# TusKANNy/seismic

Hardware: AMD Instinct MI355X
Metric: queries/sec + mean latency (µs) at fixed recall@10 vs exact, SPLADE-v3 MSMARCO (higher is better)
Workload: dtype f32

## Files before the change

include/seismic_hip_testing.h:

```cpp
#ifndef SEISMIC_HIP_TESTING_H
#define SEISMIC_HIP_TESTING_H
#include "seismic_hip.h"
#ifdef __cplusplus
extern "C" {
#endif

uint32_t sgpu_debug_host_threads(void);
uint32_t sgpu_debug_chunk_bounds(uint32_t nq, uint32_t chunk_min, uint32_t chunk_max, uint32_t lanes_free, uint32_t* bounds);
sgpu_status sgpu_debug_pack_forward(const sgpu_index* idx, uint8_t* out_fwd, uint64_t cap, uint64_t* out_doc_ref,
                                    uint64_t* out_bytes);
sgpu_status sgpu_debug_row_dir(const sgpu_index* idx, uint32_t* out, uint64_t cap_words, uint64_t* n_words, uint32_t* n_buckets);
sgpu_status sgpu_debug_plan(const sgpu_index* idx, const uint64_t* q_off, const uint32_t* comps, const float* vals,
                            uint32_t nq, uint32_t query_cut, uint32_t* order_out, uint32_t* out3);
sgpu_status sgpu_debug_device_plan(sgpu_index* idx, const uint64_t* q_off, const uint32_t* comps, const float* vals,
                                   uint32_t nq, uint32_t query_cut, uint32_t* order_out, uint32_t* out3);
void sgpu_debug_call_timing(double* buf8);
uint32_t sgpu_debug_coop_trace(sgpu_index* idx, uint64_t* out, uint32_t cap);

#ifdef __cplusplus
}
#endif
#endif
```

seismic_amd/csrc/abi.cpp:

```cpp
#include <algorithm>
#include <chrono>
#include <cstdlib>
#include <mutex>
#include <new>
#include <string>
#include <thread>
#include <vector>

#include "host_index.hpp"

struct sgpu_batch;

namespace sgpu {
struct Lane;
sgpu_status device_index_upload(const HostIndex& h, int device, DeviceIndex** out);
sgpu_status device_index_clone(const DeviceIndex* src, int device, DeviceIndex** out);
void device_index_free(DeviceIndex* d);
uint64_t device_index_bytes(const DeviceIndex* d);
Lane* lane_acquire(DeviceIndex* d);
Lane* lane_try_acquire(DeviceIndex* d);
bool call_enter(DeviceIndex* d);
void call_exit(DeviceIndex* d);
void lane_release(DeviceIndex* d, Lane* l);
Lane* lane_main(DeviceIndex* d);
sgpu_batch** lane_scratch(Lane* l);
sgpu_status batch_create(DeviceIndex* d, Lane* lane, uint64_t dim, const uint64_t* q_off, const uint32_t* comps,
                         const float* vals, uint32_t nq, uint32_t k_max, sgpu_batch** out);
void batch_free(sgpu_batch* b);
sgpu_status batch_run(DeviceIndex* d, Lane* lane, sgpu_batch* b, const sgpu_search_params& sp, uint32_t mode,
                      int sync, sgpu_launch_stats* stats);
sgpu_status batch_sync(DeviceIndex* d, sgpu_launch_stats* stats);
sgpu_status batch_fetch(DeviceIndex* d, Lane* lane, sgpu_batch* b, uint32_t k, float* out_scores, uint64_t* out_ids,
                        uint32_t* out_n);
sgpu_status batch_fetch_stats(DeviceIndex* d, sgpu_batch* b, uint32_t* out);
sgpu_status staged_launch(DeviceIndex* d, Lane* lane, uint64_t dim, const uint64_t* q_off, const uint32_t* comps,
                          const float* vals, uint32_t nq, uint32_t q_base, const sgpu_search_params& sp, sgpu_batch** slot,
                          uint32_t followed,
                          const FilterRef* flt);
sgpu_status staged_finish(DeviceIndex* d, Lane* lane, sgpu_batch* b, float* out_scores, uint64_t* out_ids, uint32_t* out_n);
sgpu_status summary_distances(DeviceIndex* d, const HostIndex& h, uint32_t list, const uint32_t* comps,
                              const float* vals, uint32_t nnz, float* out_dots, uint32_t* out_nb);
int device_count();
double*& call_timing();
bool device_plan_applies(const DeviceIndex* d, const sgpu_search_params& sp);
sgpu_status debug_device_plan(DeviceIndex* d, const uint64_t* q_off, const uint32_t* comps, const float* vals, uint32_t nq,
                              uint32_t query_cut, uint32_t* order_out, uint32_t* out3);
sgpu_status debug_plan(const HostIndex& h, const uint64_t* q_off, const uint32_t* comps, const float* vals, uint32_t nq,
                       uint32_t query_cut, uint32_t* order_out, uint32_t* out3);
uint32_t coop_trace_dump(DeviceIndex* d, uint64_t* out, uint32_t cap);
const DeviceIndex* batch_replica(const sgpu_batch* b);
sgpu_status device_index_set_knn(DeviceIndex* d, const std::vector<uint32_t>& knn, uint32_t knn_dim);
sgpu_status build_knn_on_device(DeviceIndex* d, HostIndex& h, uint32_t nknn);
sgpu_status exact_search_device(sgpu_index* idx, uint32_t replica, const uint64_t* q_off, const uint32_t* comps,
                                const float* vals, uint32_t nq, uint32_t k, float* out_scores, uint64_t* out_ids,
                                uint32_t* out_n, const sgpu_filter* filter);
sgpu_status filter_create(sgpu_index* idx, const uint32_t* doc_ids, uint64_t n, sgpu_filter** out);
const sgpu_index* filter_index(const sgpu_filter* f);
const uint32_t* filter_host_bits(const sgpu_filter* f);
uint64_t filter_count(const sgpu_filter* f);
uint64_t filter_device_bytes(const sgpu_filter* f);
void filter_destroy(sgpu_filter* f);
bool filter_build_times(const sgpu_filter* f, uint32_t replica, double* out2);
}

using namespace sgpu;

extern "C" {

const char* sgpu_last_error(void) { return last_error().c_str(); }
uint32_t sgpu_abi_version(void) { return 4; }

sgpu_status sgpu_device_count(int32_t* n) {
  if (!n) return fail(SGPU_EINVAL, "null argument");
  *n = device_count();
  if (*n <= 0) {
    *n = 0;
    return fail(SGPU_EDEVICE, "no HIP device visible");
  }
  return SGPU_OK;
}

sgpu_status sgpu_index_create(const sgpu_index_desc* desc, sgpu_index** out) {
  if (!desc || !out) return fail(SGPU_EINVAL, "null argument");
  sgpu_index* ix = new (std::nothrow) sgpu_index();
  if (!ix) return fail(SGPU_ENOMEM, "out of memory");
  sgpu_status st = host_index_from_desc(*desc, &ix->host);
  if (st != SGPU_OK) {
    delete ix;
    return st;
  }
  *out = ix;
  return SGPU_OK;
}

sgpu_status sgpu_index_build(uint32_t comp_width, uint64_t n_docs, uint64_t dim, const uint64_t* offsets,
                             const void* comps, const float* vals, const sgpu_build_config* cfg,
                             sgpu_index** out) {
  if (!offsets || !cfg || !out || (offsets[n_docs] && (!comps || !vals))) return fail(SGPU_EINVAL, "null argument");
  sgpu_index* ix = new (std::nothrow) sgpu_index();
  if (!ix) return fail(SGPU_ENOMEM, "out of memory");
  sgpu_status st = build_host_index(comp_width, n_docs, dim, offsets, comps, vals, *cfg, &ix->host);
  if (st != SGPU_OK) {
// ... 168 lines not shown
  DeviceIndex* d = replica_of(idx, replica);
  if (!d) return SGPU_EDEVICE;
  return batch_create(d, lane_main(d), idx->host.dim, q_off, comps, vals, nq, k_max, out);
}

sgpu_status sgpu_batch_create(sgpu_index* idx, const uint64_t* q_off, const uint32_t* comps, const float* vals,
                              uint32_t nq, uint32_t k_max, sgpu_batch** out) {
  return sgpu_batch_create_on(idx, 0, q_off, comps, vals, nq, k_max, out);
}

sgpu_status sgpu_batch_run(sgpu_index* idx, sgpu_batch* batch, const sgpu_search_params* params, int32_t sync,
                           sgpu_launch_stats* stats) {
  if (!idx || !batch || !params) return fail(SGPU_EINVAL, "null argument");
  DeviceIndex* d = replica_of_batch(idx, batch);
  if (!d) return SGPU_EINVAL;
  return batch_run(d, nullptr, batch, *params, 0 , sync, stats);
}

sgpu_status sgpu_batch_run_counted(sgpu_index* idx, sgpu_batch* batch, const sgpu_search_params* params,
                                   sgpu_launch_stats* stats) {
  if (!idx || !batch || !params) return fail(SGPU_EINVAL, "null argument");
  DeviceIndex* d = replica_of_batch(idx, batch);
  if (!d) return SGPU_EINVAL;
  return batch_run(d, nullptr, batch, *params, 2 , 1, stats);
}

sgpu_status sgpu_batch_sync(sgpu_index* idx, sgpu_launch_stats* stats) {
  if (!idx) return fail(SGPU_EINVAL, "null argument");
  for (size_t i = idx->replicas.size(); i-- > 1;) {
    sgpu_status st = batch_sync(idx->replicas[i], nullptr);
    if (st != SGPU_OK) return st;
  }
  return batch_sync(idx->dev, stats);
}

sgpu_status sgpu_batch_fetch(sgpu_index* idx, sgpu_batch* batch, uint32_t k, float* out_scores,
                             uint64_t* out_doc_ids, uint32_t* out_n) {
  if (!idx || !batch || !out_scores || !out_doc_ids || !out_n) return fail(SGPU_EINVAL, "null argument");
  DeviceIndex* d = replica_of_batch(idx, batch);
  if (!d) return SGPU_EINVAL;
  return batch_fetch(d, nullptr, batch, k, out_scores, out_doc_ids, out_n);
}

sgpu_status sgpu_batch_fetch_stats(sgpu_index* idx, sgpu_batch* batch, uint32_t* out_counters) {
  if (!idx || !batch || !out_counters) return fail(SGPU_EINVAL, "null argument");
  DeviceIndex* d = replica_of_batch(idx, batch);
  if (!d) return SGPU_EINVAL;
  return batch_fetch_stats(d, batch, out_counters);
}

void sgpu_batch_destroy(sgpu_batch* batch) { batch_free(batch); }

static uint32_t chunk_jobs(uint32_t nq, uint32_t chunk_min, uint32_t chunk_max) {
  return chunk_min && nq >= 2 * chunk_min ? std::min<uint32_t>(chunk_max, nq / chunk_min) : 1u;
}
static void chunk_bounds(uint32_t nq, uint32_t n_jobs, uint32_t j, uint32_t* q0, uint32_t* q1) {
  *q0 = (uint32_t)((uint64_t)nq * j / n_jobs);
  *q1 = (uint32_t)((uint64_t)nq * (j + 1) / n_jobs);
}

static sgpu_status search_shard(DeviceIndex* d, uint64_t dim, const uint64_t* q_off, const uint32_t* comps,
                                const float* vals, uint32_t nq, uint32_t q_base, const sgpu_search_params& params,
                                float* out_scores, uint64_t* out_doc_ids, uint32_t* out_n, const FilterRef* flt) {
  static const uint32_t chunk_min = [] {
    const char* v = std::getenv("SGPU_CHUNK_MIN");
    return v && *v ? (uint32_t)std::strtoul(v, nullptr, 10) : 0xffffffffu;
  }();
  struct Job {
    Lane* lane;
    uint32_t q0, q1;
  };
  static const uint32_t chunk_max_env = [] {
    const char* v = std::getenv("SGPU_CHUNK_MAX");
    const uint32_t n = v && *v ? (uint32_t)std::strtoul(v, nullptr, 10) : 0u;
    return n > 8 ? 8u : n;
  }();
  struct InFlight {
    DeviceIndex* d;
    bool shared;
    explicit InFlight(DeviceIndex* d_) : d(d_), shared(call_enter(d_)) {}
    ~InFlight() { call_exit(d); }
  } in_flight(d);
  const uint32_t chunk_max = chunk_max_env ? chunk_max_env : ((in_flight.shared || device_plan_applies(d, params)) ? 2u : 4u);
  Job jobs[8];
  const uint32_t cmin = chunk_min != 0xffffffffu ? chunk_min : (device_plan_applies(d, params) ? 1300u : 600u);
  uint32_t n_jobs = chunk_jobs(nq, cmin, chunk_max);
  std::vector<uint64_t> off;
  if (n_jobs > 1) {
    try {
      off.resize((size_t)nq / 2 + 2);
    } catch (const std::exception&) {
      n_jobs = 1;
    }
  }
  jobs[0].lane = lane_acquire(d);
  for (uint32_t j = 1; j < n_jobs; ++j) {
    jobs[j].lane = lane_try_acquire(d);
    if (!jobs[j].lane) {
      n_jobs = j;
      break;
    }
  }
  const uint32_t k = params.k;
  sgpu_status st = SGPU_OK;
  std::string msg;
  uint32_t launched = 0;
  if (n_jobs > 1) {
    uint32_t max_nnz = 0;
    st = q_off[0] != 0 ? fail(SGPU_EINVAL, "q_off[0] must be 0") : validate_query_offsets(q_off, nq, q_base, &max_nnz);
    if (st != SGPU_OK) msg = last_error();
  }
  for (uint32_t j = 0; j < n_jobs && st == SGPU_OK; ++j) {
    Job& jb = jobs[j];
    chunk_bounds(nq, n_jobs, j, &jb.q0, &jb.q1);
    const uint64_t* qo = q_off;
    if (n_jobs > 1 && jb.q0 != 0) {
      for (uint32_t q = jb.q0; q <= jb.q1; ++q) off[q - jb.q0] = q_off[q] - q_off[jb.q0];
      qo = off.data();
    }
    st = staged_launch(d, jb.lane, dim, qo, comps ? comps + q_off[jb.q0] : nullptr, vals ? vals + q_off[jb.q0] : nullptr,
                       jb.q1 - jb.q0, q_base + jb.q0, params, lane_scratch(jb.lane), j + 1 < n_jobs ? 2u : (in_flight.shared ? 1u : 0u),
                       flt);
    if (st == SGPU_OK) ++launched;
    else msg = last_error();
  }
  for (uint32_t j = 0; j < launched; ++j) {
    Job& jb = jobs[j];
    const sgpu_status fs = staged_finish(d, jb.lane, *lane_scratch(jb.lane), out_scores + (size_t)jb.q0 * k,
                                         out_doc_ids + (size_t)jb.q0 * k, out_n + jb.q0);
    if (fs != SGPU_OK && st == SGPU_OK) {
      st = fs;
      msg = last_error();
    }
  }
  for (uint32_t j = 0; j < n_jobs; ++j) lane_release(d, jobs[j].lane);
  if (st != SGPU_OK) last_error() = msg;
  return st;
}

}

static sgpu_status batch_search(sgpu_index* idx, const uint64_t* q_off, const uint32_t* comps, const float* vals,
                                uint32_t nq, const sgpu_search_params* params, float* out_scores,
                                uint64_t* out_doc_ids, uint32_t* out_n, const sgpu_filter* filter) {
  if (!idx || !params || !q_off || !out_scores || !out_doc_ids || !out_n) return fail(SGPU_EINVAL, "null argument");
  if (params->k == 0) return fail(SGPU_EINVAL, "k must be > 0 (KHeap::new asserts, reference src/utils.rs:23)");
  if (idx->replicas.empty()) return fail(SGPU_EDEVICE, "index is not uploaded to a device (call sgpu_index_upload)");
  if (q_off[nq] && (!comps || !vals)) return fail(SGPU_EINVAL, "null argument");
  const uint32_t n_rep = (uint32_t)idx->replicas.size();
  if (n_rep == 1) {
    const FilterRef fr{filter, 0};
    return search_shard(idx->dev, idx->host.dim, q_off, comps, vals, nq, 0, *params, out_scores, out_doc_ids, out_n,
                        filter ? &fr : nullptr);
  }
  if (nq < 2 * n_rep) {
    const uint32_t r = idx->next_replica.fetch_add(1, std::memory_order_relaxed) % n_rep;
    const FilterRef fr{filter, r};
    return search_shard(idx->replicas[r], idx->host.dim, q_off, comps, vals, nq, 0, *params, out_scores, out_doc_ids, out_n,
                        filter ? &fr : nullptr);
  }
  {
    uint32_t max_nnz = 0;
    if (q_off[0] != 0) return fail(SGPU_EINVAL, "q_off[0] must be 0");
    const sgpu_status vst = validate_query_offsets(q_off, nq, 0, &max_nnz);
    if (vst != SGPU_OK) return vst;
  }
  const uint32_t k = params->k;
  try {
    std::vector<sgpu_status> sts(n_rep, SGPU_OK);
    std::vector<std::string> msgs(n_rep);
    std::vector<std::vector<uint64_t>> offs(n_rep);
    for (uint32_t r = 0; r < n_rep; ++r) {
      const uint32_t q0 = (uint32_t)((uint64_t)nq * r / n_rep), q1 = (uint32_t)((uint64_t)nq * (r + 1) / n_rep);
      offs[r].resize(q1 - q0 + 1);
      for (uint32_t q = q0; q <= q1; ++q) offs[r][q - q0] = q_off[q] - q_off[q0];
    }
    auto shard = [&](uint32_t r) {
      const uint32_t q0 = (uint32_t)((uint64_t)nq * r / n_rep), q1 = (uint32_t)((uint64_t)nq * (r + 1) / n_rep);
      try {
        const FilterRef fr{filter, r};
        sts[r] = search_shard(idx->replicas[r], idx->host.dim, offs[r].data(), comps ? comps + q_off[q0] : nullptr,
                              vals ? vals + q_off[q0] : nullptr, q1 - q0, q0, *params, out_scores + (size_t)q0 * k,
                              out_doc_ids + (size_t)q0 * k, out_n + q0, filter ? &fr : nullptr);
        if (sts[r] != SGPU_OK) msgs[r] = last_error();
      } catch (const std::exception&) {
        sts[r] = SGPU_ENOMEM;
      }
    };
    std::vector<std::thread> threads;
// ... 72 lines not shown
  if (breakdown_us) slot = phases;
  const uint32_t k = params->k;
  sgpu_status st = SGPU_OK;
  const auto t0 = std::chrono::steady_clock::now();
  for (uint32_t q = 0; q < nq && st == SGPU_OK; ++q) {
    if (q_off[q + 1] < q_off[q] || q_off[q + 1] - q_off[q] > 0xffffffffull) {
      st = fail(SGPU_EINVAL, "query offsets must be monotone (query %u)", q);
      break;
    }
    const auto tq = per_query_us ? std::chrono::steady_clock::now() : t0;
    st = sgpu_search(idx, comps ? comps + q_off[q] : nullptr, vals ? vals + q_off[q] : nullptr,
                     (uint32_t)(q_off[q + 1] - q_off[q]), params, out_scores + (size_t)q * k,
                     out_doc_ids + (size_t)q * k, out_n + q);
    if (per_query_us) per_query_us[q] = std::chrono::duration<double, std::micro>(std::chrono::steady_clock::now() - tq).count();
  }
  const double total = std::chrono::duration<double, std::micro>(std::chrono::steady_clock::now() - t0).count();
  slot = saved;
  if (mean_us) *mean_us = nq ? total / nq : 0.0;
  if (breakdown_us)
    for (int i = 0; i < 8; ++i) breakdown_us[i] = nq ? phases[i] / nq : 0.0;
  return st;
}

sgpu_status sgpu_search_sequential(sgpu_index* idx, const uint64_t* q_off, const uint32_t* comps, const float* vals,
                                   uint32_t nq, const sgpu_search_params* params, float* out_scores,
                                   uint64_t* out_doc_ids, uint32_t* out_n, double* mean_us, double* breakdown_us) {
  return sgpu_search_sequential_timed(idx, q_off, comps, vals, nq, params, out_scores, out_doc_ids, out_n, mean_us,
                                      breakdown_us, nullptr);
}

static bool test_hooks_on() {
  const char* t = std::getenv("SGPU_TEST_HOOKS");
  return t && *t && *t != '0';
}
#define SGPU_HOOK_OR(ret)                                                                            \
  if (!test_hooks_on()) {                                                                            \
    (void)fail(SGPU_EINVAL, "%s is a test hook: set SGPU_TEST_HOOKS=1 (include/seismic_hip_testing.h)", __func__); \
    return ret;                                                                                      \
  }

uint32_t sgpu_debug_host_threads(void) {
  SGPU_HOOK_OR(0u);
  return (uint32_t)host_threads();
}

uint32_t sgpu_debug_chunk_bounds(uint32_t nq, uint32_t chunk_min, uint32_t chunk_max, uint32_t lanes_free, uint32_t* bounds) {
  SGPU_HOOK_OR(0u);
  uint32_t n_jobs = chunk_jobs(nq, chunk_min, chunk_max < 1 ? 1 : (chunk_max > 8 ? 8 : chunk_max));
  if (lanes_free >= 1 && n_jobs > lanes_free) n_jobs = lanes_free;
  for (uint32_t j = 0; j < n_jobs; ++j) chunk_bounds(nq, n_jobs, j, bounds + 2 * j, bounds + 2 * j + 1);
  return n_jobs;
}

sgpu_status sgpu_debug_pack_forward(const sgpu_index* idx, uint8_t* out_fwd, uint64_t cap, uint64_t* out_doc_ref, uint64_t* out_bytes) {
  SGPU_HOOK_OR(SGPU_EINVAL);
  if (!idx || !out_bytes) return fail(SGPU_EINVAL, "null argument");
  try {
    std::vector<uint8_t> raw, fwd;
    std::vector<uint64_t> off16, dref;
    pack_dvb_raw_flags(idx->host, &raw);
    pack_record_offsets(idx->host, raw, 128 / 16, &off16);
    *out_bytes = std::max<uint64_t>(off16[idx->host.n_docs] * 16, 16);
    if (!out_fwd) return SGPU_OK;
    if (cap < *out_bytes || !out_doc_ref) return fail(SGPU_EINVAL, "buffer too small");
    pack_records(idx->host, raw, off16, &fwd);
    pack_doc_refs(idx->host, raw, off16, &dref);
    std::memcpy(out_fwd, fwd.data(), fwd.size());
    std::memcpy(out_doc_ref, dref.data(), dref.size() * 8);
  } catch (const std::bad_alloc&) {
    return fail(SGPU_ENOMEM, "out of host memory");
  }
  return SGPU_OK;
}

sgpu_status sgpu_debug_row_dir(const sgpu_index* idx, uint32_t* out, uint64_t cap_words, uint64_t* n_words, uint32_t* n_buckets) {
  SGPU_HOOK_OR(SGPU_EINVAL);
  if (!idx || !n_words || !n_buckets) return fail(SGPU_EINVAL, "null argument");
  try {
    std::vector<uint16_t> mid;
    std::vector<uint32_t> dir;
    pack_row_mid(idx->host, &mid);
    *n_buckets = 0;
    if (!pack_row_dir(idx->host, mid, &dir, n_buckets)) *n_buckets = 0;
    *n_words = dir.size();
    if (!out) return SGPU_OK;
    if (cap_words < dir.size()) return fail(SGPU_EINVAL, "buffer too small");
    std::memcpy(out, dir.data(), dir.size() * 4);
  } catch (const std::bad_alloc&) {
    return fail(SGPU_ENOMEM, "out of host memory");
  }
  return SGPU_OK;
}

sgpu_status sgpu_debug_plan(const sgpu_index* idx, const uint64_t* q_off, const uint32_t* comps, const float* vals, uint32_t nq,
                            uint32_t query_cut, uint32_t* order_out, uint32_t* out3) {
  SGPU_HOOK_OR(SGPU_EINVAL);
  if (!idx || !q_off || !order_out || !out3) return fail(SGPU_EINVAL, "null argument");
  return debug_plan(idx->host, q_off, comps, vals, nq, query_cut, order_out, out3);
}

sgpu_status sgpu_debug_device_plan(sgpu_index* idx, const uint64_t* q_off, const uint32_t* comps, const float* vals, uint32_t nq,
                                   uint32_t query_cut, uint32_t* order_out, uint32_t* out3) {
  SGPU_HOOK_OR(SGPU_EINVAL);
  if (!idx || !q_off || !order_out || !out3) return fail(SGPU_EINVAL, "null argument");
  return debug_device_plan(idx->dev, q_off, comps, vals, nq, query_cut, order_out, out3);
}
// ... 60 lines not shown
```

seismic_amd/csrc/common.hpp:

```cpp
#pragma once
#include <cstdarg>
#include <cstdint>
#include <cstdio>
#include <cstring>
#include <string>

#include "../../include/seismic_hip.h"

namespace sgpu {

std::string& last_error();
sgpu_status fail(sgpu_status st, const char* fmt, ...) __attribute__((format(printf, 2, 3)));

int default_host_threads(int omp_max_threads);
}
#ifdef _OPENMP
#include <omp.h>
#endif
namespace sgpu {
inline int host_threads() {
#ifdef _OPENMP
  return default_host_threads(omp_get_max_threads());
#else
  return 1;
#endif
}

inline float f16_to_f32(uint16_t h) {
  const uint32_t sign = (uint32_t)(h & 0x8000u) << 16;
  const uint32_t em = h & 0x7fffu;
  uint32_t bits;
  if (em >= 0x7c00u) {
    bits = sign | 0x7f800000u | ((em & 0x3ffu) << 13);
  } else if (em >= 0x0400u) {
    bits = sign | ((em << 13) + 0x38000000u);
  } else if (em == 0) {
    bits = sign;
  } else {
    float f = (float)em * 5.9604644775390625e-08f;
    uint32_t fb;
    std::memcpy(&fb, &f, 4);
    bits = sign | fb;
  }
  float f;
  std::memcpy(&f, &bits, 4);
  return f;
}

inline uint16_t f32_to_f16_sat(float f) {
  uint32_t x;
  std::memcpy(&x, &f, 4);
  const uint16_t sign = (uint16_t)((x >> 16) & 0x8000u);
  x &= 0x7fffffffu;
  if (x > 0x7f800000u) return (uint16_t)(sign | 0x7e00u);
  if (x >= 0x477ff000u) return (uint16_t)(sign | 0x7bffu);
  if (x < 0x38800000u) {
    float a;
    std::memcpy(&a, &x, 4);
    float r = __builtin_nearbyintf(a * 16777216.0f);
    return (uint16_t)(sign | (uint16_t)r);
  }
  const uint32_t lsb = (x >> 13) & 1u;
  x += 0xfffu + lsb;
  return (uint16_t)(sign | (uint16_t)((x - 0x38000000u) >> 13));
}

inline int32_t total_key(float f) {
// ... 27 lines not shown
```

seismic_amd/csrc/device_index.hip:

```cpp
#include <hip/hip_runtime.h>

#include <algorithm>
#include <atomic>
#include <chrono>
#include <cmath>
#include <condition_variable>
#include <cstdlib>
#include <cstring>
#include <mutex>
#include <unordered_map>
#include <vector>

#include "device_types.hpp"
#include "filter.hpp"
#include "host_index.hpp"

namespace sgpu {

hipError_t run_u16_dense(const LaunchArgs& a, int* occupancy);
hipError_t run_u16_packed(const LaunchArgs& a, int* occupancy);
hipError_t run_u32_split(const LaunchArgs& a, int* occupancy);
hipError_t run_u32_packed(const LaunchArgs& a, int* occupancy);
hipError_t run_u32_hash(const LaunchArgs& a, int* occupancy);
hipError_t run_u16_dense_u8(const LaunchArgs& a, int* occupancy);
// ... 426 lines not shown
    if (e != hipSuccess) return bail(fail(SGPU_EDEVICE, "hipMemcpyPeerAsync %d -> %d failed: %s", src->device, device, hipGetErrorString(e)));
  }
  if (hipStreamSynchronize(d->main.stream) != hipSuccess) return bail(fail(SGPU_EDEVICE, "peer copy failed"));
  *out = d;
  return SGPU_OK;
}

}

struct sgpu_batch_plan {
  uint32_t query_cut = 0;
  uint32_t dots_cap = 1;
  uint32_t max_nb = 0;
  uint32_t max_list_nb = 1;
  std::vector<uint32_t> order;
  bool hash_ok = true;
};

struct sgpu_batch {
  std::vector<uint64_t> h_off;
  std::vector<uint32_t> h_off32;
  std::vector<uint32_t> h_comp;
  std::vector<float> h_val;
  std::vector<sgpu_batch_plan> plans;
  int device = -1;
  const sgpu::DeviceIndex* owner = nullptr;
  uint32_t nq = 0, k_max = 0, max_nnz = 0;
  uint64_t cap_nq = 0, cap_nnz = 0, cap_slab = 0;
  uint32_t* q_off = nullptr;
  uint32_t* q_comp = nullptr;
  float* q_val = nullptr;
  uint32_t* q_order = nullptr;
  uint32_t* h_order = nullptr;
  uint32_t order_cut = 0xffffffffu;
  float* out_scores = nullptr;
  uint64_t* out_ids = nullptr;
  uint32_t* out_n = nullptr;
  uint32_t* out_stats = nullptr;
  uint32_t* status = nullptr;
  size_t status_off = 0;
  bool staged = false;
  uint8_t* arena_dev = nullptr;
  uint8_t* arena_host = nullptr;
  uint8_t* arena_host_dev = nullptr;
  bool direct_out = false;
  uint32_t done_seq = 0;
  bool direct_in = false;
  uint32_t queue_base = 0;
  size_t arena_cap = 0, in_bytes = 0, out_off = 0, out_bytes = 0;
  uint32_t* queue_dev = nullptr;
  uint32_t device_plan_cut = 0xffffffffu;
  bool followed = false;
  bool plan_identity = false;
};

namespace sgpu {

}
extern char** environ;
namespace sgpu {
struct EnvCache {
  uint64_t fp = 0;
  int n = 0;
  struct E {
    const char* name;
    const char* val;
  } e[96];
};
static thread_local EnvCache tl_env;
static void env_refresh() {
  uint64_t h = 1469598103934665603ull;
  for (char** p = environ; p && *p; ++p) h = (h ^ (uint64_t)(uintptr_t)*p) * 1099511628211ull;
  if (h != tl_env.fp || tl_env.n == 0) {
    tl_env.fp = h;
    tl_env.n = 0;
  }
}
static const char* env_get(const char* name) {
  EnvCache& c = tl_env;
  for (int i = 0; i < c.n; ++i)
    if (c.e[i].name == name) return c.e[i].val;
  const char* v = std::getenv(name);
  if (c.n < (int)(sizeof(c.e) / sizeof(c.e[0]))) c.e[c.n++] = EnvCache::E{name, v};
  return v;
}
static uint32_t env_u32(const char* name, uint32_t dflt) {
  const char* v = env_get(name);
  if (!v || !*v) return dflt;
  return (uint32_t)std::strtoul(v, nullptr, 10);
}
static bool hooks_on() {
  const char* v = env_get("SGPU_TEST_HOOKS");
  return v && *v && *v != '0';
}
static void hook_ignored(const char* name) {
  static std::atomic<bool> said{false};
  const char* v = env_get(name);
  if (v && *v && !said.exchange(true))
    std::fprintf(stderr, "seismic_hip: %s is a test hook and is ignored unless SGPU_TEST_HOOKS=1 is set (further ignored hooks are not reported)\n", name);
}
static uint32_t hook_u32(const char* name, uint32_t dflt) {
  if (hooks_on()) return env_u32(name, dflt);
  hook_ignored(name);
  return dflt;
}
static const char* hook_get(const char* name) {
// ... 201 lines not shown
    pl.order.resize(2 * (size_t)nq);
    for (uint32_t i = 0; i < nq; ++i) pl.order[i] = (uint32_t)keys[i];
    pl.hash_ok = d->view.dim < (1u << 24) && d->comp_width == 4 && d->value_type == SGPU_VAL_F16 && !hook_u32("SGPU_NO_HASH", 0);
    if (pl.hash_ok) {
      std::vector<uint32_t> stamp(kHashSlots, 0xffffffffu);
      uint32_t epoch = 0;
      for (uint32_t q = 0; q < nq && pl.hash_ok; ++q) {
        const uint64_t a = h_off[q], e = h_off[q + 1];
        uint32_t seed = kHashSeeds;
        if (e - a <= kHashSlots / 4)
          for (uint32_t s = 0; s < kHashSeeds && seed == kHashSeeds; ++s) {
            const uint32_t mult = hash_mult(s);
            bool clash = false;
            for (uint64_t i = a; i < e && !clash; ++i) {
              uint32_t& slot = stamp[hash_slot(h_comp[i], mult)];
              clash = slot == epoch;
              slot = epoch;
            }
            ++epoch;
            if (!clash) seed = s;
          }
        if (seed == kHashSeeds) pl.hash_ok = false;
        pl.order[(size_t)nq + q] = seed & (kHashSeeds - 1);
      }
    }
  } catch (const std::bad_alloc&) {
    return fail(SGPU_ENOMEM, "out of host memory planning a query batch");
  }
  return SGPU_OK;
}

sgpu_status debug_plan(const HostIndex& h, const uint64_t* q_off, const uint32_t* comps, const float* vals, uint32_t nq,
                       uint32_t query_cut, uint32_t* order_out, uint32_t* out3) {
  DeviceIndex d;
  d.comp_width = h.comp_width;
  d.view.dim = (uint32_t)h.dim;
  d.list_nb.resize(h.dim);
  d.list_np.resize(h.dim);
  for (uint64_t c = 0; c < h.dim; ++c) {
    d.list_nb[c] = (uint32_t)(h.list_block_start[c + 1] - h.list_block_start[c]);
    d.list_np[c] = (uint32_t)(h.block_post_start[h.list_block_start[c + 1]] - h.block_post_start[h.list_block_start[c]]);
  }
  sgpu_batch_plan pl;
  env_refresh();
  const sgpu_status st = make_plan(&d, q_off, comps, vals, nq, query_cut, &pl);
  if (st != SGPU_OK) return st;
  for (uint32_t i = 0; i < nq; ++i) order_out[i] = pl.order[i];
  out3[0] = pl.dots_cap;
  out3[1] = pl.max_nb;
  out3[2] = pl.max_list_nb;
  return SGPU_OK;
}

bool device_plan_applies(const DeviceIndex* d, const sgpu_search_params& sp) {
  const bool hash_family = d->comp_width == 4 && d->value_type == SGPU_VAL_F16 && d->view.dim < (1u << 24);
  const char* v = std::getenv("SGPU_DEVICE_PLAN");
  return sp.query_cut >= 1 && sp.query_cut <= kDevicePlanCutMax && !sp.first_sorted && !hash_family && !(v && *v == '0');
}

sgpu_status debug_device_plan(DeviceIndex* d, const uint64_t* q_off, const uint32_t* comps, const float* vals, uint32_t nq,
                              uint32_t query_cut, uint32_t* order_out, uint32_t* out3) {
  if (!d) return fail(SGPU_EDEVICE, "index is not uploaded to a device");
  if (nq == 0 || nq > kDevicePlanMaxQueries || query_cut == 0 || query_cut > kDevicePlanCutMax)
    return fail(SGPU_EINVAL, "the device plans 1 ... %u queries at query_cut 1 ... %u", (unsigned)kDevicePlanMaxQueries, (unsigned)kDevicePlanCutMax);
  HIP_TRY(hipSetDevice(d->device));
  const uint64_t nnz = q_off[nq];
  uint32_t n2 = 2;
  while (n2 < nq) n2 <<= 1;
  std::vector<uint32_t> off32((size_t)nq + 1);
  for (uint32_t q = 0; q <= nq; ++q) off32[q] = (uint32_t)q_off[q];
  const size_t o_comp = al16_((size_t)(nq + 1) * 4), o_val = o_comp + al16_(nnz * 4), o_keys = o_val + al16_(nnz * 4),
               o_max = o_keys + (size_t)n2 * 8, o_order = o_max + 16, total = o_order + (size_t)nq * 4;
  uint8_t* buf = nullptr;
  if (hipMalloc((void**)&buf, total) != hipSuccess) return fail(SGPU_ENOMEM, "hipMalloc of %zu bytes failed", total);
  hipError_t e = hipMemcpy(buf, off32.data(), (size_t)(nq + 1) * 4, hipMemcpyHostToDevice);
  if (e == hipSuccess && nnz) e = hipMemcpy(buf + o_comp, comps, nnz * 4, hipMemcpyHostToDevice);
  if (e == hipSuccess && nnz) e = hipMemcpy(buf + o_val, vals, nnz * 4, hipMemcpyHostToDevice);
  if (e == hipSuccess) e = hipMemset(buf + o_max, 0, 16);
  if (e == hipSuccess)
    e = launch_device_plan(d->view, (const uint32_t*)buf, (const uint32_t*)(buf + o_comp), (const float*)(buf + o_val), nq, query_cut,
                           (uint64_t*)(buf + o_keys), (uint32_t*)(buf + o_max), (uint32_t*)(buf + o_order), d->main.stream);
  if (e == hipSuccess) e = hipStreamSynchronize(d->main.stream);
  if (e == hipSuccess) e = hipMemcpy(order_out, buf + o_order, (size_t)nq * 4, hipMemcpyDeviceToHost);
  if (e == hipSuccess) e = hipMemcpy(out3, buf + o_max, 12, hipMemcpyDeviceToHost);
  (void)hipFree(buf);
  if (e != hipSuccess) return fail(SGPU_EDEVICE, "device plan failed: %s", hipGetErrorString(e));
  return SGPU_OK;
}

static sgpu_status plan_for(DeviceIndex* d, sgpu_batch* b, uint32_t query_cut, const sgpu_batch_plan** out) {
  for (const auto& pl : b->plans)
    if (pl.query_cut == query_cut) {
      *out = &pl;
      return SGPU_OK;
    }
  if (b->staged) return fail(SGPU_EINVAL, "a staged batch is planned when it is staged");
  sgpu_batch_plan pl;
  sgpu_status st = make_plan(d, b->h_off.data(), b->h_comp.data(), b->h_val.data(), b->nq, query_cut, &pl);
  if (st != SGPU_OK) return st;
  try {
    b->plans.push_back(std::move(pl));
  } catch (const std::bad_alloc&) {
    return fail(SGPU_ENOMEM, "out of host memory planning a query batch");
  }
  *out = &b->plans.back();
  return SGPU_OK;
}

static bool coop_by_size(const DeviceIndex* d, uint32_t nq) {
  const char* v = env_get("SGPU_COOP_MAX_NQ");
// ... 426 lines not shown
                        uint32_t* out_n) {
  if (!d || !b) return fail(SGPU_EINVAL, "null index/batch");
  if (k == 0 || k > b->k_max) return fail(SGPU_EINVAL, "k out of range for this batch");
  if (!lane) lane = &d->main;
  HIP_TRY(hipSetDevice(d->device));
  if (b->nq == 0) {
    HIP_TRY(hipStreamSynchronize(lane->stream));
    return SGPU_OK;
  }
  if (k == b->k_max) {
    HIP_TRY(hipMemcpyAsync(out_scores, b->out_scores, (size_t)b->nq * k * 4, hipMemcpyDeviceToHost, lane->stream));
    HIP_TRY(hipMemcpyAsync(out_ids, b->out_ids, (size_t)b->nq * k * 8, hipMemcpyDeviceToHost, lane->stream));
  } else {
    HIP_TRY(hipMemcpy2DAsync(out_scores, (size_t)k * 4, b->out_scores, (size_t)b->k_max * 4, (size_t)k * 4, b->nq,
                             hipMemcpyDeviceToHost, lane->stream));
    HIP_TRY(hipMemcpy2DAsync(out_ids, (size_t)k * 8, b->out_ids, (size_t)b->k_max * 8, (size_t)k * 8, b->nq,
                             hipMemcpyDeviceToHost, lane->stream));
  }
  HIP_TRY(hipMemcpyAsync(out_n, b->out_n, (size_t)b->nq * 4, hipMemcpyDeviceToHost, lane->stream));
  HIP_TRY(hipStreamSynchronize(lane->stream));
  return coop_check_board(d, lane);
}

sgpu_status batch_fetch_stats(DeviceIndex* d, sgpu_batch* b, uint32_t* out) {
  if (!d || !b || !out) return fail(SGPU_EINVAL, "null index/batch/out");
  HIP_TRY(hipSetDevice(d->device));
  HIP_TRY(hipStreamSynchronize(d->main.stream));
  if (b->nq) HIP_TRY(hipMemcpy(out, b->out_stats, (size_t)b->nq * STATS_WORDS * 4, hipMemcpyDeviceToHost));
  return SGPU_OK;
}

uint32_t coop_trace_dump(DeviceIndex* d, uint64_t* out, uint32_t cap) {
  if (!d) return 0;
  (void)hipSetDevice(d->device);
  Lane* lanes[DeviceIndex::kPool + 1];
  int nl = 0;
  lanes[nl++] = &d->main;
  for (Lane& l : d->pool) lanes[nl++] = &l;
  for (int i = 0; i < nl; ++i) {
    Lane* l = lanes[i];
    if (!l->coop || !l->coop_trace_n) continue;
    (void)hipStreamSynchronize(l->stream);
    const uint32_t n = std::min<uint32_t>(cap, l->coop_trace_n);
    if (hipMemcpy(out, l->coop + l->coop_trace_off, (size_t)n * 8, hipMemcpyDeviceToHost) != hipSuccess) return 0;
    return n;
  }
  return 0;
}

static inline size_t al16(size_t x) { return (x + 15) & ~(size_t)15; }

sgpu_status staged_launch(DeviceIndex* d, Lane* lane, uint64_t dim, const uint64_t* q_off, const uint32_t* comps,
                          const float* vals, uint32_t nq, uint32_t q_base, const sgpu_search_params& sp, sgpu_batch** slot,
                          uint32_t followed, const FilterRef* flt) {
  if (!d) return fail(SGPU_EDEVICE, "index is not uploaded to a device (call sgpu_index_upload)");
  if (sp.k == 0) return fail(SGPU_EINVAL, "k must be > 0 (KHeap::new asserts, reference src/utils.rs:23)");
  if (sp.k > 1024) return fail(SGPU_ELIMIT, "k = %u exceeds the heap limit of 1024", sp.k);
  uint32_t max_nnz = 0;
  PhaseClock pc;
  env_refresh();
  if (!q_off || q_off[0] != 0) return fail(SGPU_EINVAL, "q_off[0] must be 0");
  sgpu_status st = validate_query_offsets(q_off, nq, q_base, &max_nnz);
  if (st != SGPU_OK) return st;
  if (q_off[nq] && (!comps || !vals)) return fail(SGPU_EINVAL, "null query arrays");
  bool validated = false;
  HIP_TRY(hipSetDevice(d->device));
  const uint64_t nnz = q_off[nq];
  const uint32_t k = sp.k;
  const size_t o_fix = 16, o_off = 32, o_comp = o_off + al16((size_t)(nq + 1) * 4), o_val = o_comp + al16(nnz * 4),
               o_order = o_val + al16(nnz * 4), o_status = o_order + al16((size_t)nq * 8),
               in_bytes = o_status + 16;
  const size_t r_n = in_bytes, r_sc = r_n + al16((size_t)nq * 4), r_id = r_sc + al16((size_t)nq * k * 4),
               total = r_id + al16((size_t)nq * k * 8);
  sgpu_batch* b = *slot;
  if (b && (!b->staged || b->owner != d || b->arena_cap < total)) {
    HIP_TRY(hipStreamSynchronize(lane->stream));
    batch_free(b);
    b = nullptr;
    *slot = nullptr;
  }
  if (!b) {
    b = new (std::nothrow) sgpu_batch();
    if (!b) return fail(SGPU_ENOMEM, "out of host memory");
    b->staged = true;
    b->device = d->device;
    b->owner = d;
    b->arena_cap = std::max<size_t>(std::min<size_t>(total * 5 / 2, total + ((size_t)64 << 20)), 1 << 16);
    if (hipMalloc((void**)&b->arena_dev, b->arena_cap) != hipSuccess ||
        hipHostMalloc((void**)&b->arena_host, b->arena_cap, hipHostMallocMapped | hipHostMallocCoherent) != hipSuccess) {
      batch_free(b);
      return fail(SGPU_ENOMEM, "allocation of a %zu-byte staging arena failed", b->arena_cap);
    }
    if (hipHostGetDevicePointer((void**)&b->arena_host_dev, b->arena_host, 0) != hipSuccess) b->arena_host_dev = nullptr;
    *slot = b;
    if (hook_raw("SGPU_DEBUG_ALLOC")) std::fprintf(stderr, "sgpu alloc: arena %p..%p\n", (void*)b->arena_dev, (void*)(b->arena_dev + b->arena_cap));
  }
  b->nq = nq;
  b->k_max = k;
  b->max_nnz = max_nnz;
  b->in_bytes = in_bytes;
  b->out_off = r_n;
  b->out_bytes = total - r_n;
  if (nq == 0) {
    b->status_off = o_status;
    return SGPU_OK;
  }
  const uint32_t direct_max = hook_u32("SGPU_DIRECT_OUT_MAX", 16);
  const uint32_t qn = std::max<uint32_t>(4, (max_nnz + 3u) & ~3u);
  const uint32_t cut = std::min<uint32_t>(sp.query_cut, qn);
  try {
    b->plans.clear();
    b->plans.emplace_back();
  } catch (const std::bad_alloc&) {
    return fail(SGPU_ENOMEM, "out of host memory planning a query batch");
  }
  b->device_plan_cut = 0xffffffffu;
  b->followed = followed != 0;
  b->plan_identity = false;
  {
    const bool hash_family = d->comp_width == 4 && d->value_type == SGPU_VAL_F16 && d->view.dim < (1u << 24);
    uint32_t seen = 0;
    if (nq >= kDevicePlanMinQueries && nq <= kDevicePlanMaxQueries && cut >= 1 && cut <= kDevicePlanCutMax && !sp.first_sorted &&
        !hash_family && env_u32("SGPU_DEVICE_PLAN", 1) && !hook_u32("SGPU_NO_LPT", 0)) {
      std::lock_guard<std::mutex> lock(d->mu);
      auto it = d->plan_dots_seen.find(cut);
      if (it != d->plan_dots_seen.end()) seen = it->second;
    }
    if (seen && nq <= direct_max) seen = 0;
    if (!seen) {
      st = validate_queries(dim, q_off, comps, vals, nq, &max_nnz, q_base);
      if (st != SGPU_OK) return st;
      validated = true;
    }
    if (seen) {
      sgpu_batch_plan& pl = b->plans.back();
      pl.query_cut = cut;
      pl.dots_cap = std::max(seen, std::max<uint32_t>(d->max_nb, 1));
      pl.max_nb = 0;
      pl.max_list_nb = std::max<uint32_t>(d->max_nb, 1);
      pl.hash_ok = false;
      pl.order.clear();
      b->device_plan_cut = cut;
      b->plan_identity = followed == 2 && hook_u32("SGPU_PLAN_IDENTITY", 1) != 0;
    } else {
      st = make_plan(d, q_off, comps, vals, nq, cut, &b->plans.back());
      if (st != SGPU_OK) return st;
      std::lock_guard<std::mutex> lock(d->mu);
      uint32_t& v = d->plan_dots_seen[cut];
      v = std::max(v, b->plans.back().dots_cap);
    }
  }
  pc.lap(0);
  uint8_t* hs = b->arena_host;
  std::memset(hs, 0, 16);
  uint32_t* h32 = (uint32_t*)(hs + o_off);
  for (uint32_t q = 0; q <= nq; ++q) h32[q] = (uint32_t)q_off[q];
  if (nnz) {
    std::memcpy(hs + o_comp, comps, nnz * 4);
    std::memcpy(hs + o_val, vals, nnz * 4);
  }
  if (b->device_plan_cut == 0xffffffffu) std::memcpy(hs + o_order, b->plans.back().order.data(), (size_t)nq * 8);
  std::memset(hs + o_status, 0, 16);
  std::memset(hs + o_fix, 0, 16);
  const uint32_t direct_in_on = env_u32("SGPU_DIRECT_IN", 1);
  b->direct_out = b->arena_host_dev != nullptr && nq <= direct_max;
  b->direct_in = b->direct_out && direct_in_on != 0;
  uint8_t* in_base = b->direct_in ? b->arena_host_dev : b->arena_dev;
  b->queue_dev = b->direct_in ? lane->queue + 16 : (uint32_t*)b->arena_dev;
  b->queue_base = 0;
  b->q_off = (uint32_t*)(in_base + o_off);
  b->q_comp = (uint32_t*)(in_base + o_comp);
  b->q_val = (float*)(in_base + o_val);
  b->q_order = (uint32_t*)(in_base + o_order);
  b->order_cut = cut;
  uint8_t* out_base = b->direct_out ? b->arena_host_dev : b->arena_dev;
  b->out_n = (uint32_t*)(out_base + r_n);
  b->out_scores = (float*)(out_base + r_sc);
  b->out_ids = (uint64_t*)(out_base + r_id);
  b->out_stats = nullptr;
  b->status_off = b->direct_out ? o_fix : o_status;
  b->status = (uint32_t*)(out_base + b->status_off);
  pc.lap(1);
  if (b->direct_in) {
    if (lane->queue_dirty) {
      HIP_TRY(hipMemsetAsync(lane->queue + 16, 0, 4, lane->stream));
      lane->queue_pos = 0;
      lane->queue_dirty = false;
    }
    b->queue_base = lane->queue_pos;
  } else {
    HIP_TRY(hipMemcpyAsync(b->arena_dev, hs, in_bytes, hipMemcpyHostToDevice, lane->stream));
    if (!validated) {
      st = validate_queries(dim, q_off, comps, vals, nq, &max_nnz, q_base);
      if (st != SGPU_OK) {
        const std::string msg = last_error();
        (void)hipStreamSynchronize(lane->stream);
        last_error() = msg;
        return st;
      }
      validated = true;
    }
  }
  const DevView* view = &d->view;
  if (flt && flt->f) {
    const FilterDeviceView* fv = nullptr;
    st = filter_view(flt->f, flt->replica, &fv);
    if (st != SGPU_OK) {
      const std::string msg = last_error();
      (void)hipStreamSynchronize(lane->stream);
      last_error() = msg;
      return st;
    }
    view = &fv->view;
    HIP_TRY(hipSetDevice(d->device));
  }
  if (!b->direct_in && b->device_plan_cut != 0xffffffffu && !b->plan_identity) {
    HIP_TRY(launch_device_plan(*view, b->q_off, b->q_comp, b->q_val, nq, cut, (uint64_t*)(b->arena_dev + r_n),
                               (uint32_t*)(b->arena_dev + o_status) + 1, b->q_order, lane->stream));
  }
  pc.lap(2);
  hipError_t he = hipSuccess;
  {
    std::lock_guard<std::mutex> lock(d->mu);
    LaunchArgs a{};
    st = configure(d, lane, b, sp, MODE_SEARCH, &a, view);
    if (st == SGPU_OK) he = launch_search(a);
    if (b->direct_in) {
      if (st == SGPU_OK && he == hipSuccess) lane->queue_pos += nq + a.grid;
      else lane->queue_dirty = true;
    }
  }
  pc.lap(3);
  if (st == SGPU_OK && he == hipSuccess && !b->direct_out)
    he = hipMemcpyAsync(hs + o_status, b->arena_dev + o_status, 16 + b->out_bytes, hipMemcpyDeviceToHost, lane->stream);
  pc.lap(4);
  if (st != SGPU_OK || he != hipSuccess) {
    (void)hipStreamSynchronize(lane->stream);
    if (st == SGPU_OK) st = fail(SGPU_EDEVICE, "launch of the search failed: %s", hipGetErrorString(he));
    return st;
  }
  return SGPU_OK;
}

sgpu_status staged_finish(DeviceIndex* d, Lane* lane, sgpu_batch* b, float* out_scores, uint64_t* out_ids, uint32_t* out_n) {
  HIP_TRY(hipSetDevice(d->device));
  PhaseClock pc;
  {
    const volatile uint32_t* done = (b && b->done_seq) ? (const volatile uint32_t*)(b->arena_host + b->status_off + 4) : nullptr;
    const hipError_t we = wait_lane(lane->stream, b ? b->nq : 0, done, b ? b->done_seq : 0u);
    if (we != hipSuccess) lane->queue_dirty = true;
    HIP_TRY(we);
  }
  pc.lap(5);
  if (!b || b->nq == 0) return SGPU_OK;
  {
    const sgpu_status cs = coop_report(d, lane, *(const volatile uint32_t*)(b->arena_host + b->status_off));
    if (cs != SGPU_OK) {
      lane->queue_dirty = true;
      return cs;
    }
  }
  if (b->device_plan_cut != 0xffffffffu) {
    const uint32_t need = ((const volatile uint32_t*)(b->arena_host + b->status_off))[1];
    std::lock_guard<std::mutex> lock(d->mu);
    uint32_t& v = d->plan_dots_seen[b->device_plan_cut];
    v = std::max(v, need);
  }
  const size_t nq = b->nq, k = b->k_max;
  const uint8_t* r = b->arena_host + b->out_off;
  std::memcpy(out_n, r, nq * 4);
  std::memcpy(out_scores, r + al16(nq * 4), nq * k * 4);
  std::memcpy(out_ids, r + al16(nq * 4) + al16(nq * k * 4), nq * k * 8);
  pc.lap(6);
  return SGPU_OK;
}

sgpu_status summary_distances(DeviceIndex* d, const HostIndex& h, uint32_t list, const uint32_t* comps,
                              const float* vals, uint32_t nnz, float* out_dots, uint32_t* out_nb) {
  if (!d) return fail(SGPU_EDEVICE, "index is not uploaded to a device (call sgpu_index_upload)");
  if (list >= h.dim) return fail(SGPU_EINVAL, "list %u >= dim", list);
  const uint32_t nb = (uint32_t)(h.list_block_start[list + 1] - h.list_block_start[list]);
  *out_nb = nb;
  if (nb == 0 || nnz == 0) {
    for (uint32_t i = 0; i < nb; ++i) out_dots[i] = 0.0f;
    return SGPU_OK;
  }
  const uint64_t q_off[2] = {0, nnz};
  sgpu_batch* b = nullptr;
  sgpu_status st = batch_create(d, &d->main, h.dim, q_off, comps, vals, 1, 1, &b);
  if (st != SGPU_OK) return st;
  sgpu_search_params sp{};
  sp.k = 1;
  sp.query_cut = list;
  sp.heap_factor = 0;
// ... 91 lines not shown
```

Baseline: 1.753 million.

## Segment large query calls and plan later chunks on host

Large query batches are now split into segments of at most 8×16384 queries, and each segment is cut into chunks bounded by a maximum chunk size, so device-plan limits are respected. Chunks after the first now build their plan on the host instead of using the device plan, unless an environment variable selects otherwise. The device-plan applicability check is refactored into a helper that returns the cached dot capacity, and plan_dots_seen is only updated for batches large enough. This adds host planning work on later chunks and changes lane concurrency for very large calls.

```diff
diff --git a/include/seismic_hip_testing.h b/include/seismic_hip_testing.h
--- a/include/seismic_hip_testing.h
+++ b/include/seismic_hip_testing.h
@@ -7,6 +7,9 @@
 
 uint32_t sgpu_debug_host_threads(void);
 uint32_t sgpu_debug_chunk_bounds(uint32_t nq, uint32_t chunk_min, uint32_t chunk_max, uint32_t lanes_free, uint32_t* bounds);
+uint32_t sgpu_debug_call_bounds(uint32_t nq, uint32_t chunk_min, uint32_t chunk_max, uint32_t lanes_free, uint32_t first_pm,
+                                uint32_t* bounds, uint32_t cap);
+uint32_t sgpu_debug_lane_chunk(sgpu_index* idx, uint32_t lane, uint32_t* info4, uint32_t* order_out, uint32_t cap);
 sgpu_status sgpu_debug_pack_forward(const sgpu_index* idx, uint8_t* out_fwd, uint64_t cap, uint64_t* out_doc_ref,
                                     uint64_t* out_bytes);
 sgpu_status sgpu_debug_row_dir(const sgpu_index* idx, uint32_t* out, uint64_t cap_words, uint64_t* n_words, uint32_t* n_buckets);
diff --git a/seismic_amd/csrc/abi.cpp b/seismic_amd/csrc/abi.cpp
--- a/seismic_amd/csrc/abi.cpp
+++ b/seismic_amd/csrc/abi.cpp
@@ -36,18 +36,19 @@
 sgpu_status staged_launch(DeviceIndex* d, Lane* lane, uint64_t dim, const uint64_t* q_off, const uint32_t* comps,
                           const float* vals, uint32_t nq, uint32_t q_base, const sgpu_search_params& sp, sgpu_batch** slot,
                           uint32_t followed,
-                          const FilterRef* flt);
+                          const FilterRef* flt, uint32_t chunk);
 sgpu_status staged_finish(DeviceIndex* d, Lane* lane, sgpu_batch* b, float* out_scores, uint64_t* out_ids, uint32_t* out_n);
 sgpu_status summary_distances(DeviceIndex* d, const HostIndex& h, uint32_t list, const uint32_t* comps,
                               const float* vals, uint32_t nnz, float* out_dots, uint32_t* out_nb);
 int device_count();
 double*& call_timing();
-bool device_plan_applies(const DeviceIndex* d, const sgpu_search_params& sp);
+uint32_t device_plan_dots(DeviceIndex* d, const sgpu_search_params& sp, uint32_t nq, uint32_t cut);
 sgpu_status debug_device_plan(DeviceIndex* d, const uint64_t* q_off, const uint32_t* comps, const float* vals, uint32_t nq,
                               uint32_t query_cut, uint32_t* order_out, uint32_t* out3);
 sgpu_status debug_plan(const HostIndex& h, const uint64_t* q_off, const uint32_t* comps, const float* vals, uint32_t nq,
                        uint32_t query_cut, uint32_t* order_out, uint32_t* out3);
 uint32_t coop_trace_dump(DeviceIndex* d, uint64_t* out, uint32_t cap);
+uint32_t debug_lane_chunk(DeviceIndex* d, uint32_t lane, uint32_t* info4, uint32_t* order_out, uint32_t cap);
 const DeviceIndex* batch_replica(const sgpu_batch* b);
 sgpu_status device_index_set_knn(DeviceIndex* d, const std::vector<uint32_t>& knn, uint32_t knn_dim);
 sgpu_status build_knn_on_device(DeviceIndex* d, HostIndex& h, uint32_t nknn);
@@ -322,16 +323,29 @@
 void sgpu_batch_destroy(sgpu_batch* batch) { batch_free(batch); }
 
 static uint32_t chunk_jobs(uint32_t nq, uint32_t chunk_min, uint32_t chunk_max) {
-  return chunk_min && nq >= 2 * chunk_min ? std::min<uint32_t>(chunk_max, nq / chunk_min) : 1u;
-}
-static void chunk_bounds(uint32_t nq, uint32_t n_jobs, uint32_t j, uint32_t* q0, uint32_t* q1) {
-  *q0 = (uint32_t)((uint64_t)nq * j / n_jobs);
-  *q1 = (uint32_t)((uint64_t)nq * (j + 1) / n_jobs);
-}
-
-static sgpu_status search_shard(DeviceIndex* d, uint64_t dim, const uint64_t* q_off, const uint32_t* comps,
-                                const float* vals, uint32_t nq, uint32_t q_base, const sgpu_search_params& params,
-                                float* out_scores, uint64_t* out_doc_ids, uint32_t* out_n, const FilterRef* flt) {
+  if (!chunk_min) return 1u;
+  const uint32_t by_rule = nq >= 2 * (uint64_t)chunk_min ? std::min<uint32_t>(chunk_max, nq / chunk_min) : 1u;
+  const uint32_t by_size = (uint32_t)std::min<uint64_t>(((uint64_t)nq + kChunkQueriesMax - 1) / kChunkQueriesMax, 8u);
+  return std::max(by_rule, by_size);
+}
+static void chunk_bounds(uint32_t nq, uint32_t n_jobs, uint32_t j, uint32_t* q0, uint32_t* q1, uint32_t first_pm = 0) {
+  if (first_pm == 0 || first_pm >= 1000 || n_jobs < 2) {
+    *q0 = (uint32_t)((uint64_t)nq * j / n_jobs);
+    *q1 = (uint32_t)((uint64_t)nq * (j + 1) / n_jobs);
+    return;
+  }
+  const uint32_t first = std::min<uint32_t>(std::max<uint32_t>((uint32_t)((uint64_t)nq * first_pm / 1000), 1u), nq - (n_jobs - 1));
+  const uint32_t rest = nq - first;
+  *q0 = j == 0 ? 0u : first + (uint32_t)((uint64_t)rest * (j - 1) / (n_jobs - 1));
+  *q1 = j == 0 ? first : first + (uint32_t)((uint64_t)rest * j / (n_jobs - 1));
+}
+static uint32_t call_segments(uint32_t nq) {
+  return (uint32_t)std::max<uint64_t>(((uint64_t)nq + 8ull * kChunkQueriesMax - 1) / (8ull * kChunkQueriesMax), 1u);
+}
+
+static sgpu_status search_segment(DeviceIndex* d, uint64_t dim, const uint64_t* q_off, const uint32_t* comps,
+                                  const float* vals, uint32_t s0, uint32_t s1, uint32_t q_base, const sgpu_search_params& params,
+                                  float* out_scores, uint64_t* out_doc_ids, uint32_t* out_n, const FilterRef* flt, bool shared) {
   static const uint32_t chunk_min = [] {
     const char* v = std::getenv("SGPU_CHUNK_MIN");
     return v && *v ? (uint32_t)std::strtoul(v, nullptr, 10) : 0xffffffffu;
@@ -345,24 +359,17 @@
     const uint32_t n = v && *v ? (uint32_t)std::strtoul(v, nullptr, 10) : 0u;
     return n > 8 ? 8u : n;
   }();
-  struct InFlight {
-    DeviceIndex* d;
-    bool shared;
-    explicit InFlight(DeviceIndex* d_) : d(d_), shared(call_enter(d_)) {}
-    ~InFlight() { call_exit(d); }
-  } in_flight(d);
-  const uint32_t chunk_max = chunk_max_env ? chunk_max_env : ((in_flight.shared || device_plan_applies(d, params)) ? 2u : 4u);
+  static const uint32_t chunk_first_pm = [] {
+    const char* t = std::getenv("SGPU_TEST_HOOKS");
+    const char* v = (t && *t && *t != '0') ? std::getenv("SGPU_CHUNK_FIRST") : nullptr;
+    return v && *v ? (uint32_t)std::strtoul(v, nullptr, 10) : 0u;
+  }();
+  const uint32_t nq = s1 - s0;
+  const bool device_plans = device_plan_dots(d, params, std::min<uint32_t>(std::max<uint32_t>(nq / 2, 1u), kChunkQueriesMax), params.query_cut) != 0;
+  const uint32_t chunk_max = chunk_max_env ? chunk_max_env : ((shared || device_plans) ? 2u : 4u);
   Job jobs[8];
-  const uint32_t cmin = chunk_min != 0xffffffffu ? chunk_min : (device_plan_applies(d, params) ? 1300u : 600u);
+  const uint32_t cmin = chunk_min != 0xffffffffu ? chunk_min : (device_plans ? 1300u : 600u);
   uint32_t n_jobs = chunk_jobs(nq, cmin, chunk_max);
-  std::vector<uint64_t> off;
-  if (n_jobs > 1) {
-    try {
-      off.resize((size_t)nq / 2 + 2);
-    } catch (const std::exception&) {
-      n_jobs = 1;
-    }
-  }
   jobs[0].lane = lane_acquire(d);
   for (uint32_t j = 1; j < n_jobs; ++j) {
     jobs[j].lane = lane_try_acquire(d);
@@ -371,26 +378,47 @@
       break;
     }
   }
+  std::vector<uint64_t> off;
+  for (;;) {
+    uint32_t longest = 0;
+    for (uint32_t j = 0; j < n_jobs; ++j) {
+      chunk_bounds(nq, n_jobs, j, &jobs[j].q0, &jobs[j].q1, chunk_first_pm);
+      jobs[j].q0 += s0;
+      jobs[j].q1 += s0;
+      if (jobs[j].q0 != 0) longest = std::max(longest, jobs[j].q1 - jobs[j].q0);
+    }
+    if (n_jobs == 1 && s0 == 0) break;
+    try {
+      off.resize((size_t)longest + 1);
+      break;
+    } catch (const std::exception&) {
+      if (n_jobs == 1) {
+        lane_release(d, jobs[0].lane);
+        return fail(SGPU_ENOMEM, "out of host memory cutting a query batch");
+      }
+      for (uint32_t j = 1; j < n_jobs; ++j) lane_release(d, jobs[j].lane);
+      n_jobs = 1;
+    }
+  }
   const uint32_t k = params.k;
   sgpu_status st = SGPU_OK;
   std::string msg;
   uint32_t launched = 0;
-  if (n_jobs > 1) {
+  if (n_jobs > 1 || s0 != 0) {
     uint32_t max_nnz = 0;
-    st = q_off[0] != 0 ? fail(SGPU_EINVAL, "q_off[0] must be 0") : validate_query_offsets(q_off, nq, q_base, &max_nnz);
+    st = q_off[0] != 0 ? fail(SGPU_EINVAL, "q_off[0] must be 0") : validate_query_offsets(q_off + s0, nq, q_base + s0, &max_nnz);
     if (st != SGPU_OK) msg = last_error();
   }
   for (uint32_t j = 0; j < n_jobs && st == SGPU_OK; ++j) {
     Job& jb = jobs[j];
-    chunk_bounds(nq, n_jobs, j, &jb.q0, &jb.q1);
     const uint64_t* qo = q_off;
-    if (n_jobs > 1 && jb.q0 != 0) {
+    if (jb.q0 != 0) {
       for (uint32_t q = jb.q0; q <= jb.q1; ++q) off[q - jb.q0] = q_off[q] - q_off[jb.q0];
       qo = off.data();
     }
     st = staged_launch(d, jb.lane, dim, qo, comps ? comps + q_off[jb.q0] : nullptr, vals ? vals + q_off[jb.q0] : nullptr,
-                       jb.q1 - jb.q0, q_base + jb.q0, params, lane_scratch(jb.lane), j + 1 < n_jobs ? 2u : (in_flight.shared ? 1u : 0u),
-                       flt);
+                       jb.q1 - jb.q0, q_base + jb.q0, params, lane_scratch(jb.lane), j + 1 < n_jobs ? 2u : (shared ? 1u : 0u),
+                       flt, j);
     if (st == SGPU_OK) ++launched;
     else msg = last_error();
   }
@@ -405,6 +433,23 @@
   }
   for (uint32_t j = 0; j < n_jobs; ++j) lane_release(d, jobs[j].lane);
   if (st != SGPU_OK) last_error() = msg;
+  return st;
+}
+
+static sgpu_status search_shard(DeviceIndex* d, uint64_t dim, const uint64_t* q_off, const uint32_t* comps,
+                                const float* vals, uint32_t nq, uint32_t q_base, const sgpu_search_params& params,
+                                float* out_scores, uint64_t* out_doc_ids, uint32_t* out_n, const FilterRef* flt) {
+  struct InFlight {
+    DeviceIndex* d;
+    bool shared;
+    explicit InFlight(DeviceIndex* d_) : d(d_), shared(call_enter(d_)) {}
+    ~InFlight() { call_exit(d); }
+  } in_flight(d);
+  const uint32_t n_seg = call_segments(nq);
+  sgpu_status st = SGPU_OK;
+  for (uint32_t s = 0; s < n_seg && st == SGPU_OK; ++s)
+    st = search_segment(d, dim, q_off, comps, vals, (uint32_t)((uint64_t)nq * s / n_seg), (uint32_t)((uint64_t)nq * (s + 1) / n_seg),
+                        q_base, params, out_scores, out_doc_ids, out_n, flt, in_flight.shared);
   return st;
 }
 
@@ -583,6 +628,33 @@
   return n_jobs;
 }
 
+uint32_t sgpu_debug_call_bounds(uint32_t nq, uint32_t chunk_min, uint32_t chunk_max, uint32_t lanes_free, uint32_t first_pm,
+                                uint32_t* bounds, uint32_t cap) {
+  SGPU_HOOK_OR(0u);
+  const uint32_t n_seg = call_segments(nq);
+  uint32_t n = 0;
+  for (uint32_t s = 0; s < n_seg; ++s) {
+    const uint32_t s0 = (uint32_t)((uint64_t)nq * s / n_seg), s1 = (uint32_t)((uint64_t)nq * (s + 1) / n_seg);
+    uint32_t n_jobs = chunk_jobs(s1 - s0, chunk_min, chunk_max < 1 ? 1 : (chunk_max > 8 ? 8 : chunk_max));
+    if (lanes_free >= 1 && n_jobs > lanes_free) n_jobs = lanes_free;
+    for (uint32_t j = 0; j < n_jobs; ++j, ++n) {
+      uint32_t q0, q1;
+      chunk_bounds(s1 - s0, n_jobs, j, &q0, &q1, first_pm);
+      if (n < cap) {
+        bounds[2 * n] = s0 + q0;
+        bounds[2 * n + 1] = s0 + q1;
+      }
+    }
+  }
+  return n;
+}
+
+uint32_t sgpu_debug_lane_chunk(sgpu_index* idx, uint32_t lane, uint32_t* info4, uint32_t* order_out, uint32_t cap) {
+  SGPU_HOOK_OR(0u);
+  if (!idx || !idx->dev || !info4) return 0u;
+  return debug_lane_chunk(idx->dev, lane, info4, order_out, cap);
+}
+
 sgpu_status sgpu_debug_pack_forward(const sgpu_index* idx, uint8_t* out_fwd, uint64_t cap, uint64_t* out_doc_ref, uint64_t* out_bytes) {
   SGPU_HOOK_OR(SGPU_EINVAL);
   if (!idx || !out_bytes) return fail(SGPU_EINVAL, "null argument");
diff --git a/seismic_amd/csrc/common.hpp b/seismic_amd/csrc/common.hpp
--- a/seismic_amd/csrc/common.hpp
+++ b/seismic_amd/csrc/common.hpp
@@ -13,6 +13,8 @@
 sgpu_status fail(sgpu_status st, const char* fmt, ...) __attribute__((format(printf, 2, 3)));
 
 int default_host_threads(int omp_max_threads);
+
+constexpr uint32_t kChunkQueriesMax = 16384;
 }
 #ifdef _OPENMP
 #include <omp.h>
diff --git a/seismic_amd/csrc/device_index.hip b/seismic_amd/csrc/device_index.hip
--- a/seismic_amd/csrc/device_index.hip
+++ b/seismic_amd/csrc/device_index.hip
@@ -502,6 +502,8 @@
   uint32_t device_plan_cut = 0xffffffffu;
   bool followed = false;
   bool plan_identity = false;
+  uint32_t q_base = 0;
+  size_t order_off = 0;
 };
 
 namespace sgpu {
@@ -809,10 +811,21 @@
   return SGPU_OK;
 }
 
-bool device_plan_applies(const DeviceIndex* d, const sgpu_search_params& sp) {
+static_assert((uint32_t)kDevicePlanMaxQueries == kChunkQueriesMax, "abi.cpp cuts calls by kChunkQueriesMax");
+uint32_t device_plan_dots(DeviceIndex* d, const sgpu_search_params& sp, uint32_t nq, uint32_t cut) {
+  env_refresh();
   const bool hash_family = d->comp_width == 4 && d->value_type == SGPU_VAL_F16 && d->view.dim < (1u << 24);
-  const char* v = std::getenv("SGPU_DEVICE_PLAN");
-  return sp.query_cut >= 1 && sp.query_cut <= kDevicePlanCutMax && !sp.first_sorted && !hash_family && !(v && *v == '0');
+  if (nq < kDevicePlanMinQueries || nq > kDevicePlanMaxQueries || cut < 1 || cut > kDevicePlanCutMax || sp.first_sorted ||
+      hash_family || !env_u32("SGPU_DEVICE_PLAN", 1) || hook_u32("SGPU_NO_LPT", 0))
+    return 0;
+  std::lock_guard<std::mutex> lock(d->mu);
+  const auto it = d->plan_dots_seen.find(cut);
+  return it != d->plan_dots_seen.end() ? it->second : 0u;
+}
+bool later_chunks_on_host() {
+  env_refresh();
+  const char* v = env_get("SGPU_CHUNK_PLAN");
+  return !(v && !std::strcmp(v, "device"));
 }
 
 sgpu_status debug_device_plan(DeviceIndex* d, const uint64_t* q_off, const uint32_t* comps, const float* vals, uint32_t nq,
@@ -1345,7 +1358,7 @@
 
 sgpu_status staged_launch(DeviceIndex* d, Lane* lane, uint64_t dim, const uint64_t* q_off, const uint32_t* comps,
                           const float* vals, uint32_t nq, uint32_t q_base, const sgpu_search_params& sp, sgpu_batch** slot,
-                          uint32_t followed, const FilterRef* flt) {
+                          uint32_t followed, const FilterRef* flt, uint32_t chunk) {
   if (!d) return fail(SGPU_EDEVICE, "index is not uploaded to a device (call sgpu_index_upload)");
   if (sp.k == 0) return fail(SGPU_EINVAL, "k must be > 0 (KHeap::new asserts, reference src/utils.rs:23)");
   if (sp.k > 1024) return fail(SGPU_ELIMIT, "k = %u exceeds the heap limit of 1024", sp.k);
@@ -1392,6 +1405,8 @@
   b->k_max = k;
   b->max_nnz = max_nnz;
   b->in_bytes = in_bytes;
+  b->q_base = q_base;
+  b->order_off = o_order;
   b->out_off = r_n;
   b->out_bytes = total - r_n;
   if (nq == 0) {
@@ -1411,14 +1426,8 @@
   b->followed = followed != 0;
   b->plan_identity = false;
   {
-    const bool hash_family = d->comp_width == 4 && d->value_type == SGPU_VAL_F16 && d->view.dim < (1u << 24);
-    uint32_t seen = 0;
-    if (nq >= kDevicePlanMinQueries && nq <= kDevicePlanMaxQueries && cut >= 1 && cut <= kDevicePlanCutMax && !sp.first_sorted &&
-        !hash_family && env_u32("SGPU_DEVICE_PLAN", 1) && !hook_u32("SGPU_NO_LPT", 0)) {
-      std::lock_guard<std::mutex> lock(d->mu);
-      auto it = d->plan_dots_seen.find(cut);
-      if (it != d->plan_dots_seen.end()) seen = it->second;
-    }
+    uint32_t seen = device_plan_dots(d, sp, nq, cut);
+    if (seen && chunk > 0 && later_chunks_on_host()) seen = 0;
     if (seen && nq <= direct_max) seen = 0;
     if (!seen) {
       st = validate_queries(dim, q_off, comps, vals, nq, &max_nnz, q_base);
@@ -1438,9 +1447,11 @@
     } else {
       st = make_plan(d, q_off, comps, vals, nq, cut, &b->plans.back());
       if (st != SGPU_OK) return st;
-      std::lock_guard<std::mutex> lock(d->mu);
-      uint32_t& v = d->plan_dots_seen[cut];
-      v = std::max(v, b->plans.back().dots_cap);
+      if (nq >= kDevicePlanMinQueries) {
+        std::lock_guard<std::mutex> lock(d->mu);
+        uint32_t& v = d->plan_dots_seen[cut];
+        v = std::max(v, b->plans.back().dots_cap);
+      }
     }
   }
   pc.lap(0);
@@ -1533,6 +1544,21 @@
     return st;
   }
   return SGPU_OK;
+}
+
+uint32_t debug_lane_chunk(DeviceIndex* d, uint32_t lane, uint32_t* info4, uint32_t* order_out, uint32_t cap) {
+  if (!d || lane >= (uint32_t)DeviceIndex::kPool) return 0;
+  std::lock_guard<std::mutex> lk(d->pool_mu);
+  const Lane& l = d->pool[lane];
+  const sgpu_batch* b = l.scratch;
+  if (l.busy || !b || !b->staged || b->nq == 0) return 0;
+  const bool host = b->device_plan_cut == 0xffffffffu;
+  info4[0] = b->nq;
+  info4[1] = b->q_base;
+  info4[2] = host ? 0u : (b->plan_identity ? 2u : 1u);
+  info4[3] = b->order_cut;
+  if (host && order_out) std::memcpy(order_out, b->arena_host + b->order_off, (size_t)std::min<uint32_t>(cap, b->nq) * 4);
+  return 1;
 }
 
 sgpu_status staged_finish(DeviceIndex* d, Lane* lane, sgpu_batch* b, float* out_scores, uint64_t* out_ids, uint32_t* out_n) {
```

New measurement: 1.783 million (median of 6 runs). 1.7% higher.
